# Blaizzy/mlx-audio

Measured on AMD Instinct MI355X. Metric: audio samples/sec + real-time factor, Kokoro-82M TTS, higher is better.
Workload: dtype bf16 weights x fp32 activations: vocoder convs = fp16 hi pass (v_mfma_f32_32x32x16_f16) + block-scaled FP4 (e2m1) lo pass (v_mfma_scale_f32_32x32x64_f8f6f4 cbsz / blgp 4, OCP MX: E8M0 scale per row x 32 channels / per output column), fp32 accumulate; front end bf16 hi+lo split; 1 GPU; Kokoro-82M bf16 TTS, tokens->waveform, canonical short sentence T=80 F=264 (6.6 s @ 24 kHz); utterances_per_gpu=64, global_batch=64, samples_per_utterance=158400, parallelism=utterance-dp1, precision_mode=6, wire=fp32

## Files before the change

### include/mi355audio.h

```cpp
#ifndef MI355AUDIO_H
#define MI355AUDIO_H

#include <stdint.h>

#ifdef __cplusplus
extern "C" {
#endif

#define MI355_OK 0
#define MI355_ERR_ARG (-1)
#define MI355_ERR_LAUNCH (-2)
#define MI355_ERR_UNSUPPORTED (-3)

const char* mi355_last_error(void);
int mi355_abi_version(void);
int mi355_device_info(int dev, char* name, int name_cap, int* cu_count, int* lds_bytes);

enum { MI355_ACT_NONE = 0, MI355_ACT_LEAKY = 1, MI355_ACT_SNAKE = 2, MI355_ACT_GELU = 3,
       MI355_ACT_ELU = 4,
       MI355_ACT_SILU = 5,
       MI355_ACT_GELU_TANH = 6,
       MI355_ACT_TANH = 7 };

typedef struct {
// ... 66 lines not shown
int mi355_pack_conv_weight_mx4_host(const float* w_host, int32_t Cout, int32_t K, int32_t Cin, uint8_t* out_host);

typedef struct {
  const float* x; int64_t x_bstride; int32_t ldx; int32_t C; int32_t L; const int32_t* lens;
  int32_t B;
  double* sums;
  const float* gb;
  int32_t gb_ld;
  float eps;
  float* scale; float* shift; int32_t out_ld;
  int32_t reuse_sums;
} mi355_adain_coef_args;
int mi355_adain_coef(const mi355_adain_coef_args* a, void* stream);

typedef struct {
  const float* partials; int64_t bstride;
  int32_t C; int32_t L; const int32_t* lens; int32_t B;
  const float* gb; int32_t gb_ld; float eps;
  float* scale; float* shift; int32_t out_ld;
} mi355_adain_partials_args;
int mi355_adain_from_partials(const mi355_adain_partials_args* a, void* stream);

typedef struct {
  const float* x; int64_t x_bstride; int32_t ldx;
  const float* res; int64_t res_bstride; int32_t ldr;
  int32_t C; int32_t L; const int32_t* lens; int32_t B;
  const float* weight; const float* bias;
  const float* ada_gb; int32_t ada_ld;
  float eps;
  int32_t post_act; float post_slope;
  float* y; int64_t y_bstride; int32_t ldy;
  int32_t y_split;
} mi355_layernorm_args;
int mi355_layernorm(const mi355_layernorm_args* a, void* stream);
int mi355_split16(const float* x, void* y, int64_t n, int32_t fmt, void* stream);

#define MI355_GN_PART_ELEMS 4096
typedef struct {
  const float* x; int64_t x_bstride; int32_t ldx;
  int32_t C; int32_t L; const int32_t* lens; int32_t B;
  double* partials; int64_t partials_bstride;
} mi355_group_norm_stats_args;
int mi355_group_norm_stats(const mi355_group_norm_stats_args* a, void* stream);

typedef struct {
  const void* partials; int64_t partials_bstride;
// ... 492 lines not shown
```

### mlx_audio_amd/csrc/conv_common.h

```cpp
#pragma once
#include <stdlib.h>
#include <type_traits>
#include "common.h"

namespace mi355conv {

__device__ __forceinline__ void glds16(const void* gsrc, void* ldst) {
  __builtin_amdgcn_global_load_lds((const __attribute__((address_space(1))) void*)gsrc,
                                   (__attribute__((address_space(3))) void*)ldst, 16, 0, 0);
}

__device__ __forceinline__ float gelu_erf(float x) { return 0.5f * x * (1.0f + erff(x * 0.70710678118654752f)); }
__device__ __forceinline__ float gelu_tanh(float x) { return 0.5f * x * (1.0f + tanhf(0.7978845608028654f * (x + 0.044715f * x * x * x))); }

template <int PREC>
__device__ __forceinline__ f32x16 mfma16(const bf16x8 a, const bf16x8 b, const f32x16 c) {
  if constexpr (PREC >= 3)
    return __builtin_amdgcn_mfma_f32_32x32x16_f16(__builtin_bit_cast(f16x8, a), __builtin_bit_cast(f16x8, b), c, 0, 0, 0);
  else
    return __builtin_amdgcn_mfma_f32_32x32x16_bf16(a, b, c, 0, 0, 0);
}
template <int PREC>
constexpr int a_images() { return (PREC == 2 || PREC == 4) ? 2 : 1; }
template <int PREC>
// ... 121 lines not shown
            else if (a.post_act == MI355_ACT_TANH) v = tanhf(v);
          } else if constexpr (EPI == 2) {
            v = v / (1.0f + expf(-v));
          } else if constexpr (EPI == 3) {
            v = gelu_tanh(v);
          }
          v = (v * cscale + rv[q]) * a.out_scale;
          if (ok[q]) {
            if (a.y_split) ((uint32_t*)yb)[(int64_t)orows[q] * a.ldy + ocol] = split16_word(v, a.y_split);
            else yb[(int64_t)orows[q] * a.ldy + ocol] = v;
          }
          if (want_stats && ok[q]) {
            sK[nf] = scnt[nf] == 0 ? v : sK[nf];
            const float d = v - sK[nf];
            s1[nf] += d;
            s2[nf] += d * d;
            ++scnt[nf];
          }

        }
      }
    }
  if constexpr (WM == MI355_STATS_ROWS) {
    if (want_stats && a.up_s == 0) {
      const int row0 = l0 + wm * WM;
      if (row0 < len_out) {
#pragma unroll
        for (int nf = 0; nf < NF; ++nf) {
          const int n = n0 + wn * WN + nf * 32 + (lane & 31);
          const float cl = (float)scnt[nf];
          const float ml = scnt[nf] ? sK[nf] + s1[nf] / cl : 0.f;
          const float vl = scnt[nf] ? s2[nf] - s1[nf] * s1[nf] / cl : 0.f;
          const float cp = __shfl_xor(cl, 32, 64), mp = __shfl_xor(ml, 32, 64), vp = __shfl_xor(vl, 32, 64);
          const float ct = cl + cp;
          const float dm = mp - ml;
          const float sum = ml * cl + mp * cp;
          const float m2 = vl + vp + (ct > 0.f ? dm * dm * cl * cp / ct : 0.f);
          if (lane < 32 && n < a.Cout)
            *(float2*)(a.stats_partial + (int64_t)b * a.stats_bstride + ((int64_t)(row0 / MI355_STATS_ROWS) * a.Cout + n) * 2) = make_float2(sum, m2);
        }
      }
    }
    if constexpr (EXT) {
      if (want_ext && a.up_s == 0) {
        const int row0 = l0 + wm * WM;
        if (row0 < len_out) {
#pragma unroll
// ... 90 lines not shown
          float amn = INFINITY, amx = -INFINITY;
#pragma unroll
          for (int mf = 0; mf < MF; ++mf)
#pragma unroll
            for (int r = 0; r < 16; ++r) {
              amn = fminf(amn, acc[MO + mf][nf][r]);
              amx = fmaxf(amx, acc[MO + mf][nf][r]);
            }
          const float e0 = (amn + bias) * oscale, e1 = (amx + bias) * oscale;
          float mn = fminf(e0, e1), mx = fmaxf(e0, e1);
          mn = fminf(mn, __shfl_xor(mn, 32, 64));
          mx = fmaxf(mx, __shfl_xor(mx, 32, 64));
          if (lane < 32)
            *(float2*)(a.ext_partial + (int64_t)b * a.ext_bstride + ((int64_t)(row0 / MI355_STATS_ROWS) * a.Cout + n) * 2) = make_float2(mn, mx);
        }
      }
    }
  }
}

template <int MF, int NF, int WM, int WN>
__device__ __forceinline__ void conv_epilogue_up_interior(const mi355_conv_gemm_args& a, f32x16 (&acc)[MF][NF], const int b, const int l0, const int n0,
                                                          const int wm, const int wn, const int lane) {
  const float oscale = a.out_scale;
  const int64_t urow = (int64_t)(l0 + wm * WM) * a.up_s - a.up_p + a.up_row_off;
  char* yw = (char*)(a.y + (int64_t)b * a.y_bstride + urow * a.ldy);
  const char* rw = a.res ? (const char*)(a.res + (int64_t)b * a.res_bstride + urow * a.ldr) : nullptr;
  const uint32_t ystep = (uint32_t)a.up_s * (uint32_t)a.ldy * 4u;
  const uint32_t rstep = (uint32_t)a.up_s * (uint32_t)a.ldr * 4u;
#pragma unroll
  for (int nf = 0; nf < NF; ++nf) {
    const int n = n0 + wn * WN + nf * 32 + (lane & 31);
    const int rph = n / a.up_cout, ocol = n - rph * a.up_cout;
    const float bias = a.bias ? a.bias[ocol] : 0.f;
    const uint32_t lrow = (uint32_t)(4 * (lane >> 5));
    const uint32_t yoff = lrow * ystep + ((uint32_t)rph * (uint32_t)a.ldy + (uint32_t)ocol) * 4u;
    const uint32_t roff = lrow * rstep + ((uint32_t)rph * (uint32_t)a.ldr + (uint32_t)ocol) * 4u;
#pragma unroll
    for (int mf = 0; mf < MF; ++mf)
#pragma unroll
      for (int h = 0; h < 2; ++h) {
        float rv[8];
#pragma unroll
        for (int q = 0; q < 8; ++q) rv[q] = 0.f;
        if (rw) {
#pragma unroll
          for (int q = 0; q < 8; ++q) {
            const int r = h * 8 + q;
            rv[q] = *(const float*)(rw + (roff + (uint32_t)(mf * 32 + (r & 3) + 8 * (r >> 2)) * rstep));
          }
        }
#pragma unroll
        for (int q = 0; q < 8; ++q) {
          const int r = h * 8 + q;
          const float v = ((acc[mf][nf][r] + bias) + rv[q]) * oscale;
          *(float*)(yw + (yoff + (uint32_t)(mf * 32 + (r & 3) + 8 * (r >> 2)) * ystep)) = v;
        }
        __builtin_amdgcn_sched_barrier(0);
      }
  }
}

}

int mi355_conv_ws4_launch(const mi355_conv_gemm_args& a, hipStream_t st, int feat, int bn = 128);
bool mi355_conv_ws4_eligible(const mi355_conv_gemm_args& a, bool vec);
```

### mlx_audio_amd/csrc/conv_gemm.hip

```cpp
#include "conv_common.h"

using namespace mi355conv;

namespace {

constexpr int kThreads = 256;

struct split_geom {
  int ksplit, cpz;
  int lo_slices;
};

template <int BM, int BN, int PREC, bool VEC, bool SPLIT = false>
__global__ __launch_bounds__(kThreads) void conv_gemm_kernel(const mi355_conv_gemm_args a, const split_geom sg) {
  constexpr int WM = BM / 2, WN = BN / 2, MF = WM / 32, NF = WN / 32;
  constexpr int BBYTES = (BN / 32) * 2048;
  extern __shared__ __attribute__((aligned(16))) char smem[];

  const int tid = threadIdx.x, lane = tid & 63, wave = tid >> 6;
  const int wm = wave >> 1, wn = wave & 1;
  const int b = SPLIT ? (int)blockIdx.z / sg.ksplit : (int)blockIdx.z, l0 = blockIdx.x * BM, n0 = blockIdx.y * BN;
  const int len_out = a.lens_out ? a.lens_out[b] : a.Lout;
  if (l0 >= len_out) return;
  const int len_in = a.lens_in ? a.lens_in[b] : a.Lin;
// ... 524 lines not shown
  MI355_REQUIRE(ap, "conv_gemm: null args");
  mi355_conv_gemm_args a = *ap;
  MI355_REQUIRE(a.x && a.w && a.y, "conv_gemm: null tensor");
  MI355_REQUIRE(a.B > 0 && a.Lout > 0 && a.Cout > 0 && a.Cin > 0 && a.K > 0, "conv_gemm: bad shape");
  MI355_REQUIRE(a.dil >= 1, "conv_gemm: dilation must be >= 1");
  MI355_REQUIRE((a.pre_scale == nullptr) == (a.pre_shift == nullptr), "conv_gemm: pre_scale/pre_shift must come together");
  MI355_REQUIRE(a.pre_act != MI355_ACT_SNAKE || a.pre_alpha, "conv_gemm: snake needs pre_alpha");
  MI355_REQUIRE(a.pre_act != MI355_ACT_GELU, "conv_gemm: gelu is an epilogue activation");
  MI355_REQUIRE(!a.pre_scale || (a.pre_ld % 4 == 0 && a.pre_ld >= ((a.Cin + 31) & ~31)),
                "conv_gemm: pre_ld must be >= Cin padded to 32 and a multiple of 4");
  MI355_REQUIRE(!a.up_s || (a.up_cout > 0 && a.Cout % a.up_cout == 0 && a.Cout / a.up_cout == a.up_s),
                "conv_gemm: polyphase store needs Cout == up_s*up_cout");
  if (a.precision == 0) a.precision = 2;
  MI355_REQUIRE(a.precision >= 1 && a.precision <= 6, "conv_gemm: precision must be 1 .. 6");
  MI355_REQUIRE((a.precision != 5 && a.precision != 6) || !a.pre_fq, "conv_gemm: precisions 5 / 6 have no quantising prologue");
  MI355_REQUIRE(!a.pre_fq || a.pre_act == MI355_ACT_NONE || a.pre_act == MI355_ACT_LEAKY || (a.pre_act == MI355_ACT_SNAKE && !a.pre_inv_beta),
                "conv_gemm: a quantising prologue (pre_fq) takes no activation, LeakyReLU or Snake");
  if (a.out_scale == 0.f) a.out_scale = 1.f;
  hipStream_t st = (hipStream_t)stream;
  static const bool novec_flat = getenv("MI355_CONV_NOVEC_FLAT") != nullptr && getenv("MI355_CONV_NOVEC_FLAT")[0] == '1';
  const bool vec = (a.flat_valid % 4 == 0) && (a.ldx % 4 == 0) && (a.x_off % 4 == 0) && (a.x_bstride % 4 == 0) &&
                   (((uintptr_t)a.x) % 16 == 0) && !(novec_flat && a.flat_valid > 0);
  if (a.stats_partial) {
    MI355_REQUIRE(a.up_s == 0, "conv_gemm: fused statistics need a plain (non-polyphase) store");
    MI355_REQUIRE(a.stats_bstride % 2 == 0 && ((uintptr_t)a.stats_partial) % 8 == 0, "conv_gemm: stats_partial must be 8-byte aligned");
  }
  int tile = a.tile;
  t_mx_lo_slices = 0;
  if (a.y_split) {
    MI355_REQUIRE(a.y_split == 2 || a.y_split == 4, "conv_gemm: y_split must be 0, 2 (bfloat16 hi | lo) or 4 (IEEE half hi | lo)");
    MI355_REQUIRE(!a.accumulate, "conv_gemm: y_split cannot accumulate into y (y holds split words)");
    a.split_ws = nullptr;
  }
  if (a.x_split) {
    MI355_REQUIRE(a.x_split == a.precision && (a.precision == 2 || a.precision == 4), "conv_gemm: x_split must equal the launch's precision, 2 or 4");
    MI355_REQUIRE(a.pre_act == MI355_ACT_NONE && !a.pre_scale && !a.pre_fq, "conv_gemm: a split input takes no prologue");
    MI355_REQUIRE(!a.ext_partial && mi355_conv_ws4_eligible(a, vec), "conv_gemm: x_split needs 16-byte aligned channels-last rows and a window of <= 192 rows "
                  "(the wave-specialised kernel)");
    static const int ws_feat_x = getenv("MI355_CONV_WS_FEAT") ? atoi(getenv("MI355_CONV_WS_FEAT")) : 0;
    const int rc = a.Cout <= 64 ? mi355_conv_ws4_launch(a, st, ws_feat_x & 3, 64) : mi355_conv_ws4_launch(a, st, tile % 10000000 == 6128128 ? ((tile / 10000000) % 10) : ws_feat_x);
    return rc;
  }
  if (a.ext_partial) {
    MI355_REQUIRE(conv_ext_supported(a), "conv_gemm: ext_partial needs a launch mi355_conv_gemm_ext_supported accepts (pre_fq, precision 2, plain store, K > 1)");
    MI355_REQUIRE(a.ext_bstride % 2 == 0 && ((uintptr_t)a.ext_partial) % 8 == 0, "conv_gemm: ext_partial must be 8-byte aligned");
    static const int ws_feat_e = getenv("MI355_CONV_WS_FEAT") ? atoi(getenv("MI355_CONV_WS_FEAT")) : 0;
    return mi355_conv_ws4_launch(a, st, ws_feat_e & 3, a.Cout <= 64 ? 64 : 128);
// ... 96 lines not shown
```

### mlx_audio_amd/csrc/conv_ws4.h

```cpp
#pragma once
#include "conv_common.h"

namespace mi355conv {

extern int g_ws4_resident;

constexpr int kWs4Threads = 512;

enum { P_NONE = 0, P_LEAKY = 1, P_SNAKE = 2, P_SNAKEBETA = 3, P_ELU = 4 };

struct ws4_geom {
  int tiles_per_item, P, NT, glog, fold;
  int nch;
  int keff;
  int tap_rows;
  int R;
  int gemm;
  int nslices;
  int bn;
  int feat;
  int total_ids;
  unsigned long long* dbg;
};

constexpr int kDbgSlots = 48;

struct tile_t { int b, l0, n0, len_out, len_in; };

__device__ __forceinline__ bool decode_tile(const mi355_conv_gemm_args& a, const ws4_geom& q, const int id, tile_t& t) {
  const int kq = id >> 3;
  const int ny = kq % q.NT;
  const int pg = kq / q.NT;
  const int glog = q.glog;
  const int p = (((((pg >> glog) << 3) + (id & 7)) << glog)) | (pg & ((1 << glog) - 1));
  if (p >= q.P) return false;
  t.b = p / q.tiles_per_item;
  t.l0 = (p - t.b * q.tiles_per_item) * 128;
  t.n0 = ny * q.bn;
  t.len_out = a.lens_out ? a.lens_out[t.b] : a.Lout;
  if (t.l0 >= t.len_out) return false;
  t.len_in = a.lens_in ? a.lens_in[t.b] : a.Lin;
  return true;
}
__device__ __forceinline__ int next_work(const mi355_conv_gemm_args& a, const ws4_geom& q, int id, tile_t& t) {
  for (id += (int)gridDim.x; id < q.total_ids; id += (int)gridDim.x)
    if (decode_tile(a, q, id, t)) return id;
  return -1;
}

template <int PREC, int PRE, int EPI, bool GEMM, bool DBG = false, int ABL = 0, int BN = 128, bool FQ = false, bool CW = true>
// ... 344 lines not shown
    if constexpr (DBG) {
      if (dbg && lane == 0 && ntile < 8) dbg[4 * ntile] = __builtin_amdgcn_s_memtime();
      if (dbg && lane == 0 && (ntile == 0 || ntile == 7)) dbg[32 + (ntile == 7)] = wall_clock64();
    }
    const char* wfrag = (const char*)a.w + ((int64_t)((n0 >> 5) + wn * NF)) * 2048 + lane * 16;
    auto wptr = [&](const int s) { return wfrag + (int64_t)(s < last_slice ? s : last_slice) * wstep; };
    bf16x8 b0[NB], b1[NB];
    if constexpr (!MXP) {
#pragma unroll
      for (int f = 0; f < NB; ++f) b0[f] = *(const bf16x8*)(wfrag + f * 1024);
    }

    f32x16 acc[MF][NF];
#pragma unroll
    for (int mf = 0; mf < MF; ++mf)
#pragma unroll
      for (int nf = 0; nf < NF; ++nf)
#pragma unroll
        for (int r = 0; r < 16; ++r) acc[mf][nf][r] = 0.f;

    float* yb = a.y + (int64_t)b * a.y_bstride;
    const float* rb = a.res ? a.res + (int64_t)b * a.res_bstride : nullptr;
    const bool interior = l0 + BM <= len_out && n0 + BN <= a.Cout;
    if ((ABL & 8) == 0 && fold && interior) {
      const char* rw = rb ? (const char*)(rb + (int64_t)(l0 + wm * WM) * a.ldr + (n0 + wn * WN)) : nullptr;
      const char* yr = (const char*)(yb + (int64_t)(l0 + wm * WM) * a.ldy + (n0 + wn * WN));
      const uint32_t rpb = (uint32_t)a.ldr * 4u, ypb = (uint32_t)a.ldy * 4u;
      const uint32_t roff = (uint32_t)(4 * hh) * rpb + (uint32_t)hl * 4u;
      const uint32_t yoff = (uint32_t)(4 * hh) * ypb + (uint32_t)hl * 4u;
#pragma unroll
      for (int mf = 0; mf < MF; ++mf)
#pragma unroll
        for (int nf = 0; nf < NF; ++nf) {
          float rv[16];
#pragma unroll
          for (int r = 0; r < 16; ++r) rv[r] = 0.f;
          if (rw) {
#pragma unroll
            for (int r = 0; r < 16; ++r) rv[r] = *(const float*)(rw + (roff + (uint32_t)(mf * 32 + (r & 3) + 8 * (r >> 2)) * rpb + (uint32_t)(nf * 128)));
          }
          if (a.accumulate) {
#pragma unroll
            for (int r = 0; r < 16; ++r) rv[r] += *(const float*)(yr + (yoff + (uint32_t)(mf * 32 + (r & 3) + 8 * (r >> 2)) * ypb + (uint32_t)(nf * 128)));
          }
#pragma unroll
          for (int r = 0; r < 16; ++r) acc[mf][nf][r] = rv[r];
        }
// ... 464 lines not shown
    }

    if constexpr ((ABL & 8) != 0) {
      float tsum = 0.f;
#pragma unroll
      for (int mf = 0; mf < MF; ++mf)
#pragma unroll
        for (int nf = 0; nf < NF; ++nf)
#pragma unroll
          for (int r = 0; r < 16; ++r) tsum += acc[mf][nf][r];
      if (tsum == 1.2345e-30f) yb[0] = tsum;
      continue;
    }
    const bool plain = a.up_s == 0 && a.post_act == MI355_ACT_NONE && (fold || (!a.res && !a.accumulate)) && !a.post_colscale && !a.y_split;
    if constexpr (COLW) {
      if (plain && interior) {
        conv_epilogue_interior<2, NF, 64, WN, FQ, MF, 0>(a, acc, b, l0, n0, 0, wn, lane);
        conv_epilogue_interior<2, NF, 64, WN, FQ, MF, 2>(a, acc, b, l0, n0, 1, wn, lane);
      } else {
        conv_epilogue<2, NF, 64, WN, EPI, FQ, MF, 0>(a, acc, b, l0, n0, 0, wn, lane, len_out, fold != 0);
        conv_epilogue<2, NF, 64, WN, EPI, FQ, MF, 2>(a, acc, b, l0, n0, 1, wn, lane, len_out, fold != 0);
      }
    } else {
      bool up_interior = false;
      if constexpr (EPI == 0 && !FQ && BN == 128 && PRE == P_LEAKY && !GEMM) {
        if (a.up_s != 0 && interior && a.post_act == MI355_ACT_NONE && !a.accumulate && !a.post_colscale && !a.y_split && !a.stats_partial && a.res_shift == 0 &&
            (a.up_cout & 31) == 0) {
          const int len_up = a.lens_up ? a.lens_up[b] : a.up_Lout;
          up_interior = (int64_t)l0 * a.up_s - a.up_p >= 0 && (int64_t)(l0 + BM - 1) * a.up_s + (a.up_s - 1) - a.up_p < len_up;
        }
      }
      if (plain && interior) conv_epilogue_interior<MF, NF, WM, WN, FQ>(a, acc, b, l0, n0, wm, wn, lane);
      else if (up_interior) conv_epilogue_up_interior<MF, NF, WM, WN>(a, acc, b, l0, n0, wm, wn, lane);
      else conv_epilogue<MF, NF, WM, WN, EPI, FQ>(a, acc, b, l0, n0, wm, wn, lane, len_out, fold != 0);
    }
    if constexpr (DBG) {
      if (dbg && lane == 0 && ntile < 8) dbg[4 * ntile + 3] = __builtin_amdgcn_s_memtime();
    }
  }
  if (!(q.feat & 1)) __builtin_amdgcn_s_setprio(0);
}

inline bool gemm_mode(const mi355_conv_gemm_args& a) { return a.K == 1 && a.Cin >= 64 && a.pre_act == MI355_ACT_NONE && !a.pre_scale && !a.pre_fq; }

template <int PREC, int PRE, int EPI, bool GEMM, bool DBG = false, int ABL = 0, int BN = 128, bool FQ = false, bool CW = true>
int launch_ws4(const mi355_conv_gemm_args& a, hipStream_t st, const int feat, unsigned long long* dbg = nullptr) {
  ws4_geom q;
  q.bn = BN;
  q.gemm = GEMM ? 1 : 0;
  const int chunks32 = (a.Cin + 31) >> 5;
  q.nslices = chunks32 * ((PREC == 5 || PREC == 6) ? a.K + ((a.K + 1) >> 1) : a.K);
  if (q.gemm) {
    q.nch = (chunks32 + 1) >> 1;
    q.keff = 2;
    q.tap_rows = 128;
    q.R = 256;
  } else {
    q.nch = chunks32;
    q.keff = a.K;
    q.tap_rows = a.dil;
    q.R = 128 + (a.K - 1) * a.dil;
  }
  MI355_REQUIRE(q.R <= (GEMM ? 256 : 192), "conv_gemm(ws4): window of %d rows exceeds %d (K=%d dil=%d)", q.R, GEMM ? 256 : 192, a.K, a.dil);
  const size_t lds = (size_t)2 * window_bytes<PREC>(q.R);
  q.tiles_per_item = (a.Lout + 127) / 128;
  q.P = a.B * q.tiles_per_item;
  q.NT = (a.Cout + BN - 1) / BN;
  q.fold = ((a.res || a.accumulate) && a.post_act == MI355_ACT_NONE && a.up_s == 0 && a.res_shift == 0 && !a.post_colscale) ? 1 : 0;
  q.glog = q.P >= 512 ? 3 : (q.P >= 256 ? 2 : (q.P >= 128 ? 1 : 0));
  q.feat = feat;
  q.dbg = dbg;
  const int per = 8 << q.glog;
  q.total_ids = ((q.P + per - 1) / per) * per * q.NT;
  static int cus = 0;
  if (cus == 0) {
    int dev = 0;
    hipDeviceProp_t prop;
    if (hipGetDevice(&dev) == hipSuccess && hipGetDeviceProperties(&prop, dev) == hipSuccess) cus = prop.multiProcessorCount;
    if (cus <= 0) cus = 256;
  }
  static const int wg_per_cu = getenv("MI355_CONV_WS_WG_PER_CU") ? atoi(getenv("MI355_CONV_WS_WG_PER_CU")) : 2;
  const int resident = g_ws4_resident > 0 ? ((g_ws4_resident + 7) / 8) * 8 : ((cus * wg_per_cu) / 8) * 8;
  const unsigned grid = (unsigned)((feat & 8) || q.total_ids <= resident ? q.total_ids : resident);
  MI355_CLEAR_ERROR();
  hipLaunchKernelGGL((conv_ws4_kernel<PREC, PRE, EPI, GEMM, DBG, ABL, BN, FQ, CW>), dim3(grid), dim3(kWs4Threads), lds, st, a, q);
  MI355_LAUNCH_CHECK("conv_gemm(ws4)");
  return MI355_OK;
}

inline int epi_family(const mi355_conv_gemm_args& a) {
  switch (a.post_act) {
// ... 37 lines not shown
```

### mlx_audio_amd/csrc/norm.hip

```cpp
#include "common.h"

namespace {

__global__ __launch_bounds__(256) void instnorm_partial_kernel(const mi355_adain_coef_args a, int rows_per_split) {
  __shared__ double red[2][32][33];
  const int tid = threadIdx.x, cg = tid & 7, rg = tid >> 3;
  const int b = blockIdx.z, c = blockIdx.x * 32 + cg * 4;
  const int len = a.lens ? a.lens[b] : a.L;
  const int r0 = blockIdx.y * rows_per_split;
  const int r1 = min(len, r0 + rows_per_split);
  double s[4] = {0, 0, 0, 0}, q[4] = {0, 0, 0, 0};
  const float* xb = a.x + (int64_t)b * a.x_bstride;
  if (c < a.C) {
    for (int l = r0 + rg; l < r1; l += 32) {
      const float4 v = *(const float4*)(xb + (int64_t)l * a.ldx + c);
      const float t[4] = {v.x, v.y, v.z, v.w};
#pragma unroll
      for (int i = 0; i < 4; ++i) { const double d = (double)t[i]; s[i] += d; q[i] += d * d; }
    }
  }
#pragma unroll
  for (int i = 0; i < 4; ++i) { red[0][rg][cg * 4 + i] = s[i]; red[1][rg][cg * 4 + i] = q[i]; }
  __syncthreads();
  if (tid < 64) {
// ... 89 lines not shown
        const float2 v0 = *(const float2*)(pb + (int64_t)e * estride), v1 = *(const float2*)(pb + (int64_t)(e + LPC) * estride);
        m2 += term(v0, e) + term(v1, e + LPC);
      }
      for (; e < nblk; e += LPC) m2 += term(*(const float2*)(pb + (int64_t)e * estride), e);
    }
  }
  red[cl][eg] = m2;
  __syncthreads();
  if (eg != 0 || c >= a.out_ld) return;
  float sc = 0.f, sh = 0.f;
  if (cok) {
    double q = 0.0;
    for (int j = 0; j < LPC; ++j) q += red[cl][j];
    double var = len > 0 ? q / (double)len : 0.0;
    if (var < 0) var = 0;
    const float rstd = 1.0f / sqrtf((float)var + a.eps);
    float g = 0.f, be = 0.f;
    if (a.gb) { g = a.gb[(int64_t)b * a.gb_ld + c]; be = a.gb[(int64_t)b * a.gb_ld + a.C + c]; }
    sc = (1.0f + g) * rstd;
    sh = be - (float)mean * sc;
  }
  a.scale[(int64_t)b * a.out_ld + c] = sc;
  a.shift[(int64_t)b * a.out_ld + c] = sh;
}

template <bool VEC, int NCH>
__global__ __launch_bounds__(256) void layernorm_kernel(const mi355_layernorm_args a) {
  const int lane = threadIdx.x & 63;
  const int64_t row = (int64_t)blockIdx.x * 4 + (threadIdx.x >> 6);
  if (row >= (int64_t)a.B * a.L) return;
  const int b = (int)(row / a.L), l = (int)(row - (int64_t)b * a.L);
  const int len = a.lens ? a.lens[b] : a.L;
  if (l >= len) return;
  const float* xr = a.x + (int64_t)b * a.x_bstride + (int64_t)l * a.ldx;
  const float* rr = a.res ? a.res + (int64_t)b * a.res_bstride + (int64_t)l * a.ldr : nullptr;
  float v[NCH][4];
  float s = 0.f;
  float4 w4[NCH], b4[NCH], g4[NCH], e4[NCH];
#pragma unroll
  for (int i = 0; i < NCH; ++i) {
    const int c = i * 256 + lane * 4;
    w4[i] = make_float4(1.f, 1.f, 1.f, 1.f); b4[i] = make_float4(0.f, 0.f, 0.f, 0.f); g4[i] = b4[i]; e4[i] = b4[i];
    if (c < a.C) {
      auto ld4 = [](const float* p) {
        if constexpr (VEC) return *(const float4*)p;
        else return make_float4(p[0], p[1], p[2], p[3]);
// ... 77 lines not shown
  MI355_REQUIRE(a.B > 0 && a.C > 0 && a.L > 0, "adain_coef: bad shape");
  MI355_REQUIRE(a.ldx % 4 == 0 && a.x_bstride % 4 == 0 && a.ldx >= ((a.C + 3) & ~3), "adain_coef: ldx must be a multiple of 4 and cover C rounded up to 4");
  MI355_REQUIRE(a.out_ld >= a.C, "adain_coef: out_ld < C");
  hipStream_t st = (hipStream_t)stream;
  if (!a.reuse_sums) {
    hipError_t e = hipMemsetAsync(a.sums, 0, sizeof(double) * 2 * (size_t)a.B * a.C, st);
    MI355_REQUIRE(e == hipSuccess, "adain_coef: memset failed: %s", hipGetErrorString(e));
    const int cblocks = (a.C + 31) / 32;
    int nsplit = (1024 + cblocks * a.B - 1) / (cblocks * a.B);
    const int max_split = (a.L + 63) / 64;
    if (nsplit > max_split) nsplit = max_split;
    if (nsplit < 1) nsplit = 1;
    const int rows = (a.L + nsplit - 1) / nsplit;
    MI355_CLEAR_ERROR();
    hipLaunchKernelGGL(instnorm_partial_kernel, dim3(cblocks, nsplit, a.B), dim3(256), 0, st, a, rows);
    MI355_LAUNCH_CHECK("instnorm_partial");
  }
  MI355_CLEAR_ERROR();
  hipLaunchKernelGGL(adain_finalize_kernel, dim3((a.out_ld + 127) / 128, a.B), dim3(128), 0, st, a);
  MI355_LAUNCH_CHECK("adain_finalize");
  return MI355_OK;
}

extern "C" int mi355_adain_from_partials(const mi355_adain_partials_args* ap, void* stream) {
  MI355_REQUIRE(ap && ap->partials && ap->scale && ap->shift, "adain_from_partials: null tensor");
  const mi355_adain_partials_args a = *ap;
  MI355_REQUIRE(a.B > 0 && a.C > 0 && a.L > 0 && a.out_ld >= a.C, "adain_from_partials: bad shape");
  MI355_CLEAR_ERROR();
  MI355_REQUIRE(a.bstride % 2 == 0 && ((uintptr_t)a.partials) % 8 == 0, "adain_from_partials: partials must be 8-byte aligned");
  static const int cpw_env = getenv("MI355_ADAIN_CPW") ? atoi(getenv("MI355_ADAIN_CPW")) : 0;
  if (a.B >= 8 && cpw_env != 4) hipLaunchKernelGGL(adain_from_partials_kernel<16>, dim3((a.out_ld + 15) / 16, a.B), dim3(256), 0, (hipStream_t)stream, a);
  else hipLaunchKernelGGL(adain_from_partials_kernel<4>, dim3((a.out_ld + 3) / 4, a.B), dim3(256), 0, (hipStream_t)stream, a);
  MI355_LAUNCH_CHECK("adain_from_partials");
  return MI355_OK;
}

extern "C" int mi355_layernorm(const mi355_layernorm_args* ap, void* stream) {
  MI355_REQUIRE(ap && ap->x && ap->y, "layernorm: null tensor");
  const mi355_layernorm_args a = *ap;
  MI355_REQUIRE(a.C > 0 && a.C <= 2048 && a.C % 4 == 0, "layernorm: C must be a multiple of 4 and <= 2048 (got %d)", a.C);
  MI355_REQUIRE(a.ldx % 4 == 0 && a.ldy % 4 == 0 && a.x_bstride % 4 == 0 && a.y_bstride % 4 == 0, "layernorm: strides must be multiples of 4");
  MI355_REQUIRE(!a.res || (a.ldr % 4 == 0 && a.res_bstride % 4 == 0), "layernorm: residual strides must be multiples of 4");
  MI355_REQUIRE(a.y_split == 0 || a.y_split == 2 || a.y_split == 4, "layernorm: y_split must be 0, 2 or 4");
  const int64_t rows = (int64_t)a.B * a.L;
  MI355_CLEAR_ERROR();
  const bool vec = ((uintptr_t)a.weight % 16 == 0) && ((uintptr_t)a.bias % 16 == 0) && ((uintptr_t)a.ada_gb % 16 == 0) && (a.ada_ld % 4 == 0);
// ... 12 lines not shown
```

### mlx_audio_amd/ops.py

```python
from __future__ import annotations

import ctypes
import math
import os
from dataclasses import dataclass
from typing import Optional, Tuple

import numpy as np
import torch

from . import _lib

ACT_NONE, ACT_LEAKY, ACT_SNAKE, ACT_GELU, ACT_ELU, ACT_SILU, ACT_GELU_TANH, ACT_TANH = 0, 1, 2, 3, 4, 5, 6, 7

PROFILE = None


def _stream() -> int:
    return torch.cuda.current_stream().cuda_stream


def profile_finalize(entries):
    torch.cuda.synchronize()
    out = []
# ... 458 lines not shown
def fake_quant_extrema_from_partials(ext: torch.Tensor, L: int, *, lens=None, pre=None, pre_act: int = ACT_NONE, pre_slope: float = 0.0,
                                     pre_alpha: Optional[torch.Tensor] = None) -> torch.Tensor:
    B, nblk, C, two = ext.shape
    assert two == 2 and ext.is_contiguous() and nblk >= (L + STATS_ROWS - 1) // STATS_ROWS
    mm = torch.empty((B, 2), dtype=torch.float32, device=ext.device)
    sc, sh = pre if pre is not None else (None, None)
    _lib.call_struct("mi355_fake_quant_extrema_from_partials", "mi355_fake_quant_args", _stream(), x=_ptr(ext), x_bstride=ext.stride(0), ldx=2 * C, C=C, L=L,
                     lens=_ptr(lens), B=B, pre_scale=_ptr(sc), pre_shift=_ptr(sh), pre_ld=sc.stride(0) if sc is not None else 0, pre_act=pre_act,
                     pre_slope=pre_slope, pre_alpha=_ptr(pre_alpha), minmax=_ptr(mm))
    return mm


def adain_from_partials(stats: torch.Tensor, L: int, gb: Optional[torch.Tensor], lens: Optional[torch.Tensor] = None, eps: float = 1e-5):
    B, _, C, _ = stats.shape
    cp = round_up(C, 32)
    scale = torch.empty((B, cp), dtype=torch.float32, device=stats.device)
    shift = torch.empty((B, cp), dtype=torch.float32, device=stats.device)
    _lib.call_struct("mi355_adain_from_partials", "mi355_adain_partials_args", _stream(), partials=_ptr(stats), bstride=stats.stride(0),
                     C=C, L=L, lens=_ptr(lens), B=B, gb=_ptr(gb), gb_ld=0 if gb is None else gb.stride(0), eps=eps,
                     scale=_ptr(scale), shift=_ptr(shift), out_ld=cp)
    return scale, shift


GN_PART_ELEMS = 4096


def group_norm_stats(x: torch.Tensor, lens: Optional[torch.Tensor] = None) -> torch.Tensor:
    B, L, C, xbs, ldx = _nlc(x)
    assert x.dtype == torch.float32
    parts = torch.empty((B, (L * C + GN_PART_ELEMS - 1) // GN_PART_ELEMS, 2), dtype=torch.float64, device=x.device)
    _lib.call_struct("mi355_group_norm_stats", "mi355_group_norm_stats_args", _stream(), x=_ptr(x), x_bstride=xbs, ldx=ldx, C=C, L=L, lens=_ptr(lens), B=B,
                     partials=_ptr(parts), partials_bstride=parts.stride(0))
    return parts


def group_norm_coef(partials: torch.Tensor, L: int, C: int, weight: Optional[torch.Tensor], bias: Optional[torch.Tensor], *, eps: float = 1e-5,
                    lens: Optional[torch.Tensor] = None, rep: int = 1, return_stats: bool = False):
    conv = partials.dim() == 4
    assert partials.is_contiguous() and partials.dtype == (torch.float32 if conv else torch.float64)
    assert (partials.shape[2] == C and partials.shape[3] == 2) if conv else partials.shape[2] == 2
    B = partials.shape[0]
    ld = round_up(rep * C, 32)
    scale = torch.empty((B, ld), dtype=torch.float32, device=partials.device)
    shift = torch.empty((B, ld), dtype=torch.float32, device=partials.device)
    mr = torch.empty((B, 2), dtype=torch.float32, device=partials.device) if return_stats else None
    _lib.call_struct("mi355_group_norm_coef", "mi355_group_norm_coef_args", _stream(), partials=_ptr(partials), partials_bstride=partials.stride(0),
# ... 625 lines not shown
```

### mlx_audio_amd/tts/models/kokoro/engine.py

```python
from __future__ import annotations

import math
import os
from dataclasses import dataclass, field
from typing import Dict, List, Optional, Sequence

import numpy as np
import torch

from .... import ops
from ....ops import ACT_GELU, ACT_GELU_TANH, ACT_LEAKY, ACT_NONE, ACT_SNAKE, PackedConv, round_up


def fold_weight_norm(v: torch.Tensor, g: torch.Tensor, param_dtype: torch.dtype) -> torch.Tensor:
    v_ = v.to(param_dtype)
    g_ = g.to(param_dtype)
    axes = tuple(range(1, v_.dim()))
    nrm = torch.sqrt((v_ * v_).sum(dim=axes, keepdim=True))
    w = (v_ / (nrm + torch.tensor(1e-7, dtype=param_dtype))) * g_
    return w.to(torch.float32)


@dataclass
class _AdaIN:
# ... 645 lines not shown
                                  quant=bool(self.qmods) and self._isq(f"{g_n}.m_source.l_linear"), coarse_f32=self.coarse_f32)
        nb2 = self.n_fft + 2
        nbp = ops.round_up(nb2, 4)
        n_har = L2 * up // self.hop + 1
        har = self._new(B, n_har, nbp, zero=True)[:, :, :nb2]
        lens_samples = frames * (2 * up) if ragged else None
        ops.stft_magphase(har_src, self.n_fft, self.hop, self.window, har, lens=lens_samples)
        if "har" in overrides:
            har.copy_(overrides["har"].to(device=dev, dtype=torch.float32))
        lens_har = lens_samples // self.hop + 1 if ragged else None
        x = xg
        L = L2
        lens_x = lens_2f
        nk = len(self.rk)
        for i, (u, k) in enumerate(zip(self.rates, self.kers)):
            last = i + 1 == len(self.rates)
            cout = self.ups[i].cout // u
            Lo = L * u + (1 if last else 0)
            lens_o = (lens_x * u + (1 if last else 0)) if ragged else None
            xsrc = self._new(B, Lo, cout)
            har_i = har
            if self.qmods and self._isq(f"{g_n}.noise_convs.{i}"):
                har_i = ops.fake_quant_u8(har, y=self._new(B, n_har, nbp, zero=True)[:, :, :nb2], lens=lens_har)
            if not last:
                sf = int(np.prod(self.rates[i + 1:]))
                self._conv(har_i, self.noise_convs[i], xsrc, lens_in=lens_har, lens_out=lens_o,
                           flat=dict(ldx=sf * nbp, x_off=-((sf + 1) // 2) * nbp, channels=nbp))
            else:
                self._conv(har_i, self.noise_convs[i], xsrc, lens_in=lens_har, lens_out=lens_o)
            if return_intermediates:
                trace[f"nconv{i}"] = xsrc.clone()
            xsrc = self._resblock1_fwd(self.noise_res[i], xsrc, gb_dec, lens_o)
            if return_intermediates:
                trace[f"nres{i}"] = xsrc.clone()
            kp = k // u
            xu = self._new(B, Lo, cout)
            lens_gemm = (lens_x + (kp - 1)) if ragged else None
            lens_ct = (lens_x * u) if ragged else None
            self._convq(f"{g_n}.ups.{i}", x, self.ups[i], xu, pad=kp - 1, lout=L + kp - 1, lens_in=lens_x, lens_out=lens_gemm, pre_act=ACT_LEAKY,
                        pre_slope=0.1, res=xsrc, up=dict(s=u, p=(k - u) // 2, cout=cout, row_off=1 if last else 0, lout=L * u, lens=lens_ct))
            if last:
                xu[:, 0, :].copy_(xsrc[:, 0, :])
            if return_intermediates:
                trace[f"xu{i}"] = xu.clone()
            acc = self._new(B, Lo, cout)
            xu_sums = torch.empty(B * cout * 2, dtype=torch.float64, device=dev)
            for j in range(nk):
                self._resblock1_fwd(self.resblocks[i * nk + j], xu, gb_dec, lens_o, out=acc, accumulate=j > 0,
                                    out_scale=(1.0 / nk) if j == nk - 1 else 1.0, x_sums=(xu_sums, j > 0))
            x, L, lens_x = acc, Lo, lens_o
            if return_intermediates:
                trace[f"stage{i}"] = acc.clone()
        post = self._new(B, L, round_up(nb2, 4))
        self._convq(f"{g_n}.conv_post", x, self.conv_post, post[:, :, :nb2], pad=3, lens_in=lens_x, lens_out=lens_x, pre_act=ACT_LEAKY, pre_slope=0.01)
        audio = self._new(B, (L - 1) * self.hop, zero=True)
        ops.istft_head(post[:, :, :nb2], self.n_fft, self.hop, self.window, audio, lens=lens_x)
        outs = [audio[b, : Fs[b] * 2 * up] for b in range(B)]
        durs = [dur[b, : Ts[b]] for b in range(B)]
        if return_intermediates:
            return outs, durs, dict(d=d, en=en, f0=f0_curve, n=n_curve, asr=asr, t_en=t_en, dur_raw=dur_raw, har_src=har_src,
                                    har=har, bert=h, xg=xg, post=post[:, :, :nb2], dec3=xg, **trace)
        return outs, durs
```

Measured before the change: 197.1 million samples/s.

## Fuse instance-norm statistics into polyphase upsample conv epilogue

Lets the transposed-conv (polyphase upsample) epilogue emit per-block mean/M2 partials. A new kernel reduces those partials into per-channel double sums, which lets the resblocks skip recomputing instance-norm sums over the upsampled tensor. The residual add now preloads into the accumulators rather than running in the up-interior store, and the noise-conv on the last stage also emits fused stats. The cost is extra epilogue arithmetic, an extra small reduction launch, and more complex ragged-length masking logic.

```diff
diff --git a/include/mi355audio.h b/include/mi355audio.h
--- a/include/mi355audio.h
+++ b/include/mi355audio.h
@@ -112,6 +112,17 @@
 int mi355_adain_from_partials(const mi355_adain_partials_args* a, void* stream);
 
 typedef struct {
+  const float* partials; int64_t bstride;
+  int32_t C;
+  int32_t Lg; const int32_t* lens_g;
+  int32_t up_s; int32_t up_p; int32_t up_row_off; int32_t up_Lout; const int32_t* lens_up;
+  const float* head; int64_t head_bstride; int32_t head_ld;
+  int32_t B;
+  double* sums;
+} mi355_instnorm_partials_args;
+int mi355_instnorm_sums_from_partials(const mi355_instnorm_partials_args* a, void* stream);
+
+typedef struct {
   const float* x; int64_t x_bstride; int32_t ldx;
   const float* res; int64_t res_bstride; int32_t ldr;
   int32_t C; int32_t L; const int32_t* lens; int32_t B;
diff --git a/mlx_audio_amd/csrc/conv_common.h b/mlx_audio_amd/csrc/conv_common.h
--- a/mlx_audio_amd/csrc/conv_common.h
+++ b/mlx_audio_amd/csrc/conv_common.h
@@ -167,7 +167,7 @@
       }
     }
   if constexpr (WM == MI355_STATS_ROWS) {
-    if (want_stats && a.up_s == 0) {
+    if (want_stats) {
       const int row0 = l0 + wm * WM;
       if (row0 < len_out) {
 #pragma unroll
@@ -304,43 +304,51 @@
 template <int MF, int NF, int WM, int WN>
 __device__ __forceinline__ void conv_epilogue_up_interior(const mi355_conv_gemm_args& a, f32x16 (&acc)[MF][NF], const int b, const int l0, const int n0,
                                                           const int wm, const int wn, const int lane) {
+  static_assert(WM == MI355_STATS_ROWS, "the wave block is the statistics block (2 x 2 consumer layout)");
   const float oscale = a.out_scale;
+  const bool want_stats = a.stats_partial != nullptr;
   const int64_t urow = (int64_t)(l0 + wm * WM) * a.up_s - a.up_p + a.up_row_off;
   char* yw = (char*)(a.y + (int64_t)b * a.y_bstride + urow * a.ldy);
-  const char* rw = a.res ? (const char*)(a.res + (int64_t)b * a.res_bstride + urow * a.ldr) : nullptr;
   const uint32_t ystep = (uint32_t)a.up_s * (uint32_t)a.ldy * 4u;
-  const uint32_t rstep = (uint32_t)a.up_s * (uint32_t)a.ldr * 4u;
-#pragma unroll
-  for (int nf = 0; nf < NF; ++nf) {
-    const int n = n0 + wn * WN + nf * 32 + (lane & 31);
-    const int rph = n / a.up_cout, ocol = n - rph * a.up_cout;
-    const float bias = a.bias ? a.bias[ocol] : 0.f;
-    const uint32_t lrow = (uint32_t)(4 * (lane >> 5));
-    const uint32_t yoff = lrow * ystep + ((uint32_t)rph * (uint32_t)a.ldy + (uint32_t)ocol) * 4u;
-    const uint32_t roff = lrow * rstep + ((uint32_t)rph * (uint32_t)a.ldr + (uint32_t)ocol) * 4u;
-#pragma unroll
-    for (int mf = 0; mf < MF; ++mf)
-#pragma unroll
-      for (int h = 0; h < 2; ++h) {
-        float rv[8];
-#pragma unroll
-        for (int q = 0; q < 8; ++q) rv[q] = 0.f;
-        if (rw) {
-#pragma unroll
-          for (int q = 0; q < 8; ++q) {
-            const int r = h * 8 + q;
-            rv[q] = *(const float*)(rw + (roff + (uint32_t)(mf * 32 + (r & 3) + 8 * (r >> 2)) * rstep));
-          }
-        }
-#pragma unroll
-        for (int q = 0; q < 8; ++q) {
-          const int r = h * 8 + q;
-          const float v = ((acc[mf][nf][r] + bias) + rv[q]) * oscale;
+  auto body = [&](auto stats_tag) {
+    constexpr bool STATS = decltype(stats_tag)::value;
+#pragma unroll
+    for (int nf = 0; nf < NF; ++nf) {
+      const int nb = n0 + wn * WN + nf * 32;
+      const int rph = nb / a.up_cout, ocol = nb - rph * a.up_cout + (lane & 31);
+      const float bias = a.bias ? a.bias[ocol] : 0.f;
+      const uint32_t yoff = (uint32_t)(4 * (lane >> 5)) * ystep + ((uint32_t)rph * (uint32_t)a.ldy + (uint32_t)ocol) * 4u;
+      float sK = 0.f, s1 = 0.f, s2 = 0.f;
+#pragma unroll
+      for (int mf = 0; mf < MF; ++mf) {
+#pragma unroll
+        for (int r = 0; r < 16; ++r) {
+          const float v = (acc[mf][nf][r] + bias) * oscale;
           *(float*)(yw + (yoff + (uint32_t)(mf * 32 + (r & 3) + 8 * (r >> 2)) * ystep)) = v;
+          if constexpr (STATS) {
+            if (mf == 0 && r == 0) sK = v;
+            const float d = v - sK;
+            s1 += d;
+            s2 += d * d;
+          }
         }
         __builtin_amdgcn_sched_barrier(0);
       }
-  }
+      if constexpr (STATS) {
+        const float cl = (float)(MF * 16);
+        const float ml = sK + s1 / cl;
+        const float vl = s2 - s1 * s1 / cl;
+        const float mp = __shfl_xor(ml, 32, 64), vp = __shfl_xor(vl, 32, 64);
+        const float dm = mp - ml;
+        const float sum = ml * cl + mp * cl;
+        const float m2 = vl + vp + dm * dm * cl * cl / (cl + cl);
+        if (lane < 32)
+          *(float2*)(a.stats_partial + (int64_t)b * a.stats_bstride + ((int64_t)((l0 + wm * WM) / MI355_STATS_ROWS) * a.Cout + nb + lane) * 2) = make_float2(sum, m2);
+      }
+    }
+  };
+  if (want_stats) body(std::true_type{});
+  else body(std::false_type{});
 }
 
 }
diff --git a/mlx_audio_amd/csrc/conv_gemm.hip b/mlx_audio_amd/csrc/conv_gemm.hip
--- a/mlx_audio_amd/csrc/conv_gemm.hip
+++ b/mlx_audio_amd/csrc/conv_gemm.hip
@@ -570,7 +570,6 @@
   const bool vec = (a.flat_valid % 4 == 0) && (a.ldx % 4 == 0) && (a.x_off % 4 == 0) && (a.x_bstride % 4 == 0) &&
                    (((uintptr_t)a.x) % 16 == 0) && !(novec_flat && a.flat_valid > 0);
   if (a.stats_partial) {
-    MI355_REQUIRE(a.up_s == 0, "conv_gemm: fused statistics need a plain (non-polyphase) store");
     MI355_REQUIRE(a.stats_bstride % 2 == 0 && ((uintptr_t)a.stats_partial) % 8 == 0, "conv_gemm: stats_partial must be 8-byte aligned");
   }
   int tile = a.tile;
diff --git a/mlx_audio_amd/csrc/conv_ws4.h b/mlx_audio_amd/csrc/conv_ws4.h
--- a/mlx_audio_amd/csrc/conv_ws4.h
+++ b/mlx_audio_amd/csrc/conv_ws4.h
@@ -21,11 +21,15 @@
   int feat;
   int total_ids;
   unsigned long long* dbg;
+  int up_ok;
 };
 
 constexpr int kDbgSlots = 48;
 
 struct tile_t { int b, l0, n0, len_out, len_in; };
+
+template <int PREC, int PRE, int EPI, bool GEMM, int BN, bool FQ>
+constexpr bool up_interior_inst() { return EPI == 0 && !FQ && BN == 128 && PRE == P_LEAKY && !GEMM; }
 
 __device__ __forceinline__ bool decode_tile(const mi355_conv_gemm_args& a, const ws4_geom& q, const int id, tile_t& t) {
   const int kq = id >> 3;
@@ -416,7 +420,28 @@
     float* yb = a.y + (int64_t)b * a.y_bstride;
     const float* rb = a.res ? a.res + (int64_t)b * a.res_bstride : nullptr;
     const bool interior = l0 + BM <= len_out && n0 + BN <= a.Cout;
-    if ((ABL & 8) == 0 && fold && interior) {
+    constexpr bool UPI = up_interior_inst<PREC, PRE, EPI, GEMM, BN, FQ>();
+    bool up_interior = false;
+    if constexpr (UPI && !COLW) {
+      if (q.up_ok && interior) {
+        const int len_up = a.lens_up ? a.lens_up[b] : a.up_Lout;
+        up_interior = (int64_t)l0 * a.up_s - a.up_p >= 0 && (int64_t)(l0 + BM - 1) * a.up_s + (a.up_s - 1) - a.up_p < len_up;
+      }
+    }
+    if (UPI && !COLW && (ABL & 8) == 0 && up_interior && a.res) {
+      const char* rw = (const char*)(rb + ((int64_t)(l0 + wm * WM) * a.up_s - a.up_p + a.up_row_off) * a.ldr);
+      const uint32_t rstep = (uint32_t)a.up_s * (uint32_t)a.ldr * 4u;
+#pragma unroll
+      for (int nf = 0; nf < NF; ++nf) {
+        const int nb = n0 + wn * WN + nf * 32;
+        const int rph = nb / a.up_cout, ocol = nb - rph * a.up_cout + hl;
+        const uint32_t roff = (uint32_t)(4 * hh) * rstep + ((uint32_t)rph * (uint32_t)a.ldr + (uint32_t)ocol) * 4u;
+#pragma unroll
+        for (int mf = 0; mf < MF; ++mf)
+#pragma unroll
+          for (int r = 0; r < 16; ++r) acc[mf][nf][r] = *(const float*)(rw + (roff + (uint32_t)(mf * 32 + (r & 3) + 8 * (r >> 2)) * rstep));
+      }
+    } else if ((ABL & 8) == 0 && fold && interior) {
       const char* rw = rb ? (const char*)(rb + (int64_t)(l0 + wm * WM) * a.ldr + (n0 + wn * WN)) : nullptr;
       const char* yr = (const char*)(yb + (int64_t)(l0 + wm * WM) * a.ldy + (n0 + wn * WN));
       const uint32_t rpb = (uint32_t)a.ldr * 4u, ypb = (uint32_t)a.ldy * 4u;
@@ -927,14 +952,6 @@
         conv_epilogue<2, NF, 64, WN, EPI, FQ, MF, 2>(a, acc, b, l0, n0, 1, wn, lane, len_out, fold != 0);
       }
     } else {
-      bool up_interior = false;
-      if constexpr (EPI == 0 && !FQ && BN == 128 && PRE == P_LEAKY && !GEMM) {
-        if (a.up_s != 0 && interior && a.post_act == MI355_ACT_NONE && !a.accumulate && !a.post_colscale && !a.y_split && !a.stats_partial && a.res_shift == 0 &&
-            (a.up_cout & 31) == 0) {
-          const int len_up = a.lens_up ? a.lens_up[b] : a.up_Lout;
-          up_interior = (int64_t)l0 * a.up_s - a.up_p >= 0 && (int64_t)(l0 + BM - 1) * a.up_s + (a.up_s - 1) - a.up_p < len_up;
-        }
-      }
       if (plain && interior) conv_epilogue_interior<MF, NF, WM, WN, FQ>(a, acc, b, l0, n0, wm, wn, lane);
       else if (up_interior) conv_epilogue_up_interior<MF, NF, WM, WN>(a, acc, b, l0, n0, wm, wn, lane);
       else conv_epilogue<MF, NF, WM, WN, EPI, FQ>(a, acc, b, l0, n0, wm, wn, lane, len_out, fold != 0);
@@ -972,6 +989,10 @@
   q.P = a.B * q.tiles_per_item;
   q.NT = (a.Cout + BN - 1) / BN;
   q.fold = ((a.res || a.accumulate) && a.post_act == MI355_ACT_NONE && a.up_s == 0 && a.res_shift == 0 && !a.post_colscale) ? 1 : 0;
+  q.up_ok = 0;
+  if constexpr (up_interior_inst<PREC, PRE, EPI, GEMM, BN, FQ>() && !((PREC == 5 || PREC == 6) && CW)) {
+    q.up_ok = (a.up_s != 0 && !a.accumulate && a.post_act == MI355_ACT_NONE && !a.post_colscale && a.res_shift == 0 && !a.y_split && (a.up_cout & 31) == 0) ? 1 : 0;
+  }
   q.glog = q.P >= 512 ? 3 : (q.P >= 256 ? 2 : (q.P >= 128 ? 1 : 0));
   q.feat = feat;
   q.dbg = dbg;
diff --git a/mlx_audio_amd/csrc/norm.hip b/mlx_audio_amd/csrc/norm.hip
--- a/mlx_audio_amd/csrc/norm.hip
+++ b/mlx_audio_amd/csrc/norm.hip
@@ -135,6 +135,71 @@
   }
   a.scale[(int64_t)b * a.out_ld + c] = sc;
   a.shift[(int64_t)b * a.out_ld + c] = sh;
+}
+
+__global__ __launch_bounds__(256) void instnorm_sums_from_partials_kernel(const mi355_instnorm_partials_args a) {
+  constexpr int CPW = 16, LPC = 16;
+  __shared__ double red[2][CPW][LPC + 1];
+  const int cl = threadIdx.x % CPW, eg = threadIdx.x / CPW;
+  const int c = blockIdx.x * CPW + cl, b = blockIdx.y;
+  const int lg = a.lens_g ? a.lens_g[b] : a.Lg;
+  const int lu = a.lens_up ? a.lens_up[b] : a.up_Lout;
+  const int S = a.up_s > 0 ? a.up_s : 1;
+  const int nblk = lg > 0 ? (lg + MI355_STATS_ROWS - 1) / MI355_STATS_ROWS : 0;
+  const int nent = nblk * S;
+  const bool cok = c < a.C;
+  const float* pb = a.partials + (int64_t)b * a.bstride + (int64_t)(cok ? c : 0) * 2;
+  const int64_t estride = (int64_t)S * a.C * 2;
+  auto count = [&](const int j, int64_t& off) {
+    const int e = j / S, ph = j - e * S;
+    off = (int64_t)e * estride + (int64_t)ph * a.C * 2;
+    int u0 = e * MI355_STATS_ROWS, u1 = min(u0 + MI355_STATS_ROWS, lg) - 1;
+    if (a.up_s > 0) {
+      const int d = a.up_p - ph;
+      const int lo = d > 0 ? (d + S - 1) / S : 0;
+      const int num = lu - 1 + d;
+      const int hi = num >= 0 ? num / S : -1;
+      u0 = max(u0, lo);
+      u1 = min(u1, hi);
+    }
+    return max(u1 - u0 + 1, 0);
+  };
+  double s = 0.0, q = 0.0;
+  if (cok) {
+    for (int j0 = eg; j0 < nent; j0 += 4 * LPC) {
+      float2 v[4];
+      int cnt[4];
+#pragma unroll
+      for (int i = 0; i < 4; ++i) {
+        const int j = j0 + i * LPC;
+        int64_t off;
+        cnt[i] = count(j < nent ? j : nent - 1, off);
+        if (j >= nent) cnt[i] = 0;
+        v[i] = *(const float2*)(pb + off);
+      }
+#pragma unroll
+      for (int i = 0; i < 4; ++i) {
+        const double sv = cnt[i] > 0 ? (double)v[i].x : 0.0, mv = cnt[i] > 0 ? (double)v[i].y : 0.0;
+        s += sv;
+        q += mv + sv * sv / (double)(cnt[i] > 0 ? cnt[i] : 1);
+      }
+    }
+    if (eg == 0 && a.up_s > 0 && a.head) {
+      for (int r = 0; r < a.up_row_off; ++r) {
+        const double v = (double)a.head[(int64_t)b * a.head_bstride + (int64_t)r * a.head_ld + c];
+        s += v;
+        q += v * v;
+      }
+    }
+  }
+  red[0][cl][eg] = s;
+  red[1][cl][eg] = q;
+  __syncthreads();
+  if (eg != 0 || !cok) return;
+  double st = 0.0, qt = 0.0;
+  for (int j = 0; j < LPC; ++j) { st += red[0][cl][j]; qt += red[1][cl][j]; }
+  a.sums[((int64_t)b * a.C + c) * 2] = st;
+  a.sums[((int64_t)b * a.C + c) * 2 + 1] = qt;
 }
 
 template <bool VEC, int NCH>
@@ -258,6 +323,18 @@
   return MI355_OK;
 }
 
+extern "C" int mi355_instnorm_sums_from_partials(const mi355_instnorm_partials_args* ap, void* stream) {
+  MI355_REQUIRE(ap && ap->partials && ap->sums, "instnorm_sums_from_partials: null tensor");
+  const mi355_instnorm_partials_args a = *ap;
+  MI355_REQUIRE(a.B > 0 && a.C > 0 && a.Lg > 0, "instnorm_sums_from_partials: bad shape");
+  MI355_REQUIRE(a.up_s >= 0 && a.up_p >= 0 && a.up_row_off >= 0 && (a.up_s == 0 || a.up_Lout > 0), "instnorm_sums_from_partials: bad polyphase geometry");
+  MI355_REQUIRE(a.bstride % 2 == 0 && ((uintptr_t)a.partials) % 8 == 0, "instnorm_sums_from_partials: partials must be 8-byte aligned");
+  MI355_CLEAR_ERROR();
+  hipLaunchKernelGGL(instnorm_sums_from_partials_kernel, dim3((a.C + 15) / 16, a.B), dim3(256), 0, (hipStream_t)stream, a);
+  MI355_LAUNCH_CHECK("instnorm_sums_from_partials");
+  return MI355_OK;
+}
+
 extern "C" int mi355_adain_from_partials(const mi355_adain_partials_args* ap, void* stream) {
   MI355_REQUIRE(ap && ap->partials && ap->scale && ap->shift, "adain_from_partials: null tensor");
   const mi355_adain_partials_args a = *ap;
diff --git a/mlx_audio_amd/ops.py b/mlx_audio_amd/ops.py
--- a/mlx_audio_amd/ops.py
+++ b/mlx_audio_amd/ops.py
@@ -504,6 +504,26 @@
     return scale, shift
 
 
+def instnorm_sums_from_partials(stats: torch.Tensor, C: int, L: int, lens: Optional[torch.Tensor] = None, up: Optional[dict] = None,
+                                head: Optional[torch.Tensor] = None, sums: Optional[torch.Tensor] = None) -> torch.Tensor:
+    B, nblk, Cg, two = stats.shape
+    S = up["s"] if up is not None else 1
+    assert two == 2 and stats.dtype == torch.float32 and stats.is_contiguous() and Cg == S * C and nblk >= (L + STATS_ROWS - 1) // STATS_ROWS
+    if sums is None:
+        sums = torch.empty(B * C * 2, dtype=torch.float64, device=stats.device)
+    kw = {}
+    if up is not None:
+        assert up["cout"] == C
+        kw.update(up_s=S, up_p=up["p"], up_row_off=up.get("row_off", 0), up_Lout=up["lout"], lens_up=_ptr(up.get("lens")))
+        if head is not None and up.get("row_off", 0) > 0:
+            _, Lh, Ch, hbs, ldh = _nlc(head)
+            assert Ch >= C and Lh >= up["row_off"]
+            kw.update(head=_ptr(head), head_bstride=hbs, head_ld=ldh)
+    _lib.call_struct("mi355_instnorm_sums_from_partials", "mi355_instnorm_partials_args", _stream(), partials=_ptr(stats), bstride=stats.stride(0),
+                     C=C, Lg=L, lens_g=_ptr(lens), B=B, sums=_ptr(sums), **kw)
+    return sums
+
+
 GN_PART_ELEMS = 4096
 
 
diff --git a/mlx_audio_amd/tts/models/kokoro/engine.py b/mlx_audio_amd/tts/models/kokoro/engine.py
--- a/mlx_audio_amd/tts/models/kokoro/engine.py
+++ b/mlx_audio_amd/tts/models/kokoro/engine.py
@@ -691,32 +691,42 @@
             har_i = har
             if self.qmods and self._isq(f"{g_n}.noise_convs.{i}"):
                 har_i = ops.fake_quant_u8(har, y=self._new(B, n_har, nbp, zero=True)[:, :, :nb2], lens=lens_har)
+            st_src = ops.new_stats(B, Lo, cout, dev) if (self.fuse_stats and last) else None
             if not last:
                 sf = int(np.prod(self.rates[i + 1:]))
-                self._conv(har_i, self.noise_convs[i], xsrc, lens_in=lens_har, lens_out=lens_o,
+                self._conv(har_i, self.noise_convs[i], xsrc, lens_in=lens_har, lens_out=lens_o, stats=st_src,
                            flat=dict(ldx=sf * nbp, x_off=-((sf + 1) // 2) * nbp, channels=nbp))
             else:
-                self._conv(har_i, self.noise_convs[i], xsrc, lens_in=lens_har, lens_out=lens_o)
+                self._conv(har_i, self.noise_convs[i], xsrc, lens_in=lens_har, lens_out=lens_o, stats=st_src)
             if return_intermediates:
                 trace[f"nconv{i}"] = xsrc.clone()
-            xsrc = self._resblock1_fwd(self.noise_res[i], xsrc, gb_dec, lens_o)
+                trace[f"lens{i}"] = lens_o
+                if st_src is not None:
+                    trace[f"nconv{i}_stats"] = st_src
+            xsrc = self._resblock1_fwd(self.noise_res[i], xsrc, gb_dec, lens_o, x_stats=st_src)
             if return_intermediates:
                 trace[f"nres{i}"] = xsrc.clone()
             kp = k // u
             xu = self._new(B, Lo, cout)
             lens_gemm = (lens_x + (kp - 1)) if ragged else None
             lens_ct = (lens_x * u) if ragged else None
+            up_geo = dict(s=u, p=(k - u) // 2, cout=cout, row_off=1 if last else 0, lout=L * u, lens=lens_ct)
+            st_up = ops.new_stats(B, L + kp - 1, u * cout, dev) if self.fuse_stats else None
             self._convq(f"{g_n}.ups.{i}", x, self.ups[i], xu, pad=kp - 1, lout=L + kp - 1, lens_in=lens_x, lens_out=lens_gemm, pre_act=ACT_LEAKY,
-                        pre_slope=0.1, res=xsrc, up=dict(s=u, p=(k - u) // 2, cout=cout, row_off=1 if last else 0, lout=L * u, lens=lens_ct))
+                        pre_slope=0.1, res=xsrc, up=up_geo, stats=st_up)
             if last:
                 xu[:, 0, :].copy_(xsrc[:, 0, :])
             if return_intermediates:
                 trace[f"xu{i}"] = xu.clone()
             acc = self._new(B, Lo, cout)
             xu_sums = torch.empty(B * cout * 2, dtype=torch.float64, device=dev)
+            if st_up is not None:
+                ops.instnorm_sums_from_partials(st_up, cout, L + kp - 1, lens_gemm, up=up_geo, head=xu, sums=xu_sums)
+                if return_intermediates:
+                    trace[f"xu{i}_sums"] = xu_sums
             for j in range(nk):
                 self._resblock1_fwd(self.resblocks[i * nk + j], xu, gb_dec, lens_o, out=acc, accumulate=j > 0,
-                                    out_scale=(1.0 / nk) if j == nk - 1 else 1.0, x_sums=(xu_sums, j > 0))
+                                    out_scale=(1.0 / nk) if j == nk - 1 else 1.0, x_sums=(xu_sums, j > 0 or st_up is not None))
             x, L, lens_x = acc, Lo, lens_o
             if return_intermediates:
                 trace[f"stage{i}"] = acc.clone()
```

New measurement: 200.7 million samples/s (median of 6 runs). 1.8% higher.
